# tyiannak/pyAudioAnalysis

Hardware: AMD Instinct MI355X
Metric: short-term frames/sec (34-feat, 16 kHz, 50 ms/25 ms) + HBM GB/s vs peak (higher is better)
Workload: dtype f64

## Files before the change

### pyaudioanalysis_amd/csrc/lib_host_api.hpp

```cpp
#pragma once
constexpr long long kRangedMinFrames = 65536;

static int run_host_st(const void *packed, const int64_t *offsets, int64_t n_clips, int sample_kind, double fs,
                       int window, int step, int deltas, double *out, const int64_t *out_offsets,
                       int64_t mid_ratio, int64_t mid_step, double *mid_out, const int64_t *mid_out_offsets) {
    if (!packed || !offsets) return fail(PAA_ERR_ARG, "null signal");
    { const int rc0 = ensure_init(); if (rc0) return rc0; }
    LaneGuard lane;
    const bool want_mid = mid_out != nullptr;
    if (want_mid && !deltas) return fail(PAA_ERR_ARG, "mid-term features are defined over the 68 delta rows");
    if (want_mid && mid_step < 1)
        return fail(PAA_ERR_ARG, "mid_step / short_step rounds to %lld: the reference loops forever "
                    "(MidTermFeatures.py:102,124)", (long long)mid_step);
    paa_plan *plan = nullptr;
    int rc;
    const long long frames_1 = (n_clips == 1) ? paa_num_frames(offsets[1] - offsets[0], window, step) : 0;
    const bool ranged = n_clips == 1 && out && !out_offsets && !want_mid && frames_1 >= kRangedMinFrames;
    {
        std::lock_guard<std::mutex> lk(g_mu);
        rc = plan_build(offsets, n_clips, sample_kind, fs, window, step, deltas, 0, &plan, ranged ? kCopyRanges : 1);
    }
    if (rc) return rc;
    std::unique_ptr<paa_plan, void (*)(paa_plan *)> guard(plan, plan_free_synced);
    const size_t esz = sample_kind == 0 ? 2 : (sample_kind == 2 ? 4 : 8);
    const long long base = offsets[0], n_total = offsets[n_clips] - base;
    if (base != 0) {
        for (auto &cd : plan->clips) cd.sample_off -= base;
        HIP_TRY(hipMemcpy(plan->d_clips, plan->clips.data(), plan->clips.size() * sizeof(ClipDev), hipMemcpyHostToDevice));
        std::vector<StatChunk> chunks;
        for (int64_t c = 0; c < n_clips; ++c)
            for (int i = 0; i < plan->clips[c].stat_count; ++i) {
                StatChunk ch; ch.start = plan->clips[c].sample_off + (long long)i * plan->stat_chunk;
                ch.len = (int)std::min<long long>(plan->stat_chunk, plan->clips[c].n - (long long)i * plan->stat_chunk);
                ch.clip = (int)c;
                chunks.push_back(ch);
            }
        if (!chunks.empty())
            HIP_TRY(hipMemcpy(plan->d_chunks, chunks.data(), chunks.size() * sizeof(StatChunk), hipMemcpyHostToDevice));
    }
    {
        std::lock_guard<std::mutex> lk(g_mu);
        if ((rc = scratch_reserve(lane.l->in, (size_t)n_total * esz + 64))) return rc;
        if ((rc = scratch_reserve(lane.l->out, (size_t)plan->out_doubles * 8))) return rc;
    }
    HIP_TRY(hipMemcpyAsync(lane.l->in.p, (const char *)packed + (size_t)base * esz, (size_t)n_total * esz,
                           hipMemcpyHostToDevice, cs()));
    const void *d_samples = lane.l->in.p;
    if (ranged && !plan->tiles_host.empty()) {
        double *d_out = (double *)lane.l->out.p;
        const long long T = plan->clips[0].T;
        const int F = plan->P.F;
        struct CopyStreamGuard { hipStream_t s; ~CopyStreamGuard() { if (s) (void)hipStreamSynchronize(s); } } copy_guard{lane.l->copy_stream};
        {
            std::lock_guard<std::mutex> lk(g_mu);
            if ((rc = launch_stats(plan, d_samples))) return rc;
        }
        long long first = 0;
        long long t_begin[kCopyRanges + 1];
        int used = 0;
        for (int r = 0; r < kCopyRanges && first < plan->n_tiles; ++r) {
            const long long t_target = (r == kCopyRanges - 1) ? T : T * (r + 1) / kCopyRanges;
            long long last = first;
            while (last < plan->n_tiles && (long long)plan->tiles_host[(size_t)last].t0 < t_target) ++last;
            if (last == first) continue;
            t_begin[used] = plan->tiles_host[(size_t)first].t0;
            {
                std::lock_guard<std::mutex> lk(g_mu);
                rc = kFamilies[plan->fam.family].execute(plan, d_samples, d_out, plan->d_tiles + first, last - first);
            }
            if (rc) return rc;
            HIP_TRY(hipEventRecord(lane.l->range_done[used], cs()));
            first = last;
            ++used;
        }
        t_begin[used] = T;
        for (int r = 0; r < used; ++r) {
            const long long a = t_begin[r], b = t_begin[r + 1];
            HIP_TRY(hipStreamWaitEvent(lane.l->copy_stream, lane.l->range_done[r], 0));
            HIP_TRY(hipMemcpy2DAsync(out + a, (size_t)T * 8, d_out + a, (size_t)T * 8, (size_t)(b - a) * 8, (size_t)F,
                                     hipMemcpyDeviceToHost, lane.l->copy_stream));
        }
        HIP_TRY(hipStreamSynchronize(lane.l->copy_stream));
        HIP_TRY(hipStreamSynchronize(cs()));
        return PAA_OK;
    }
    if ((rc = paa_plan_execute(plan, d_samples, (double *)lane.l->out.p))) return rc;
    if (want_mid) {
        const long long md = paa_plan_mid_doubles(plan, mid_step);
        {
            std::lock_guard<std::mutex> lk(g_mu);
            if ((rc = scratch_reserve(lane.l->mid, (size_t)md * 8))) return rc;
        }
        if ((rc = paa_plan_mid_execute(plan, (const double *)lane.l->out.p, mid_ratio, mid_step, (double *)lane.l->mid.p))) return rc;
        long long o = 0;
        for (int64_t c = 0; c < n_clips; ++c) {
            const long long cnt = 2LL * plan->P.F * paa_num_mid_windows(plan->clips[c].T, mid_step);
            double *dst = mid_out + (mid_out_offsets ? mid_out_offsets[c] : o);
            HIP_TRY(hipMemcpyAsync(dst, (double *)lane.l->mid.p + o, (size_t)cnt * 8, hipMemcpyDeviceToHost, cs()));
            o += cnt;
        }
    }
    if (out) {
        if (!out_offsets) {
            HIP_TRY(hipMemcpyAsync(out, lane.l->out.p, (size_t)plan->out_doubles * 8, hipMemcpyDeviceToHost, cs()));
        } else {
            int64_t c = 0;
            while (c < n_clips) {
                int64_t e = c;
                long long cnt = 0;
                while (e < n_clips && out_offsets[e] - out_offsets[c] == plan->clips[e].out_off - plan->clips[c].out_off) {
                    cnt = plan->clips[e].out_off - plan->clips[c].out_off + (long long)plan->P.F * plan->clips[e].T;
                    ++e;
                }
                HIP_TRY(hipMemcpyAsync(out + out_offsets[c], (double *)lane.l->out.p + plan->clips[c].out_off,
                                       (size_t)cnt * 8, hipMemcpyDeviceToHost, cs()));
                c = e;
            }
        }
    }
    HIP_TRY(hipStreamSynchronize(cs()));
    return PAA_OK;
}

extern "C" int paa_st_features_i16(const int16_t *signal, int64_t n, double fs, int window, int step, int deltas,
                                   double *out) {
    if (!out) return fail(PAA_ERR_ARG, "null out");
    const int64_t off[2] = {0, n};
    return run_host_st(signal, off, 1, 0, fs, window, step, deltas, out, nullptr, 0, 0, nullptr, nullptr);
}
extern "C" int paa_st_features_f64(const double *signal, int64_t n, double fs, int window, int step, int deltas,
                                   double *out) {
    if (!out) return fail(PAA_ERR_ARG, "null out");
    const int64_t off[2] = {0, n};
    return run_host_st(signal, off, 1, 1, fs, window, step, deltas, out, nullptr, 0, 0, nullptr, nullptr);
}
extern "C" int paa_st_features_stereo_i16(const int16_t *interleaved, int64_t n, double fs, int window, int step,
                                          int deltas, double *out) {
    if (!out) return fail(PAA_ERR_ARG, "null out");
// ... 190 lines not shown
```

### pyaudioanalysis_amd/csrc/lib_plan.hpp

```cpp
#pragma once
#ifndef PAA_STAT_CHUNK
#define PAA_STAT_CHUNK 131072
#endif
constexpr int kStatChunk = PAA_STAT_CHUNK;
static int stat_chunk_for(long long total_samples, int num_cu) {
    const long long blocks = (total_samples + kStatChunk - 1) / kStatChunk;
    if (blocks < num_cu) {
        const long long len = ((total_samples + 4LL * num_cu - 1) / (4LL * num_cu) + 63) / 64 * 64;
        return (int)std::min<long long>(kStatChunk, std::max<long long>(len, 4096));
    }
    const long long want = (blocks + num_cu - 1) / num_cu * num_cu;
    const long long len = ((total_samples + want - 1) / want + 63) / 64 * 64;
    return (int)std::min<long long>(kStatChunk, std::max<long long>(len, 4096));
}

static int choose_run_cap(const std::vector<ClipDev> &clips, int quantum, int min_run, int max_run, int halo, int wg_runs,
                          int num_cu, int shrink = 0) {
    std::map<long long, long long> hist;
    for (const ClipDev &c : clips)
        if (c.T > 0) ++hist[c.T];
    if (hist.empty()) return max_run;
    long long best_cost = -1;
    int best = max_run;
    for (int cap = max_run / quantum * quantum; cap >= min_run; cap -= quantum) {
// ... 19 lines not shown

static bool balanced_runs(const std::vector<ClipDev> &clips, int run, int quantum, int shrink, int wg_runs, int num_cu, int min_run,
                          std::vector<std::vector<int>> &lens) {
    if (wg_runs < 2 || quantum < 1 || shrink < 0 || (shrink > 0 && shrink >= quantum)) return false;
    long long total = 0, runs = 0;
    std::vector<long long> need(clips.size(), 0);
    for (size_t c = 0; c < clips.size(); ++c) {
        const long long T = clips[c].T;
        if (T <= 0) continue;
        total += T;
        const long long len = clip_run_length(T, run, quantum), later = std::max<long long>(len - shrink, 1);
        need[c] = (T <= len) ? 1 : 1 + (T - len + later - 1) / later;
        runs += need[c];
    }
    const long long slots = (long long)num_cu * wg_runs;
    if (runs >= slots || (runs + wg_runs - 1) / wg_runs > num_cu || total < slots * min_run) return false;
    std::vector<long long> k(clips.size(), 0);
    long long given = 0;
    for (size_t c = 0; c < clips.size(); ++c) {
        const long long T = clips[c].T;
        if (T <= 0) continue;
        k[c] = std::max<long long>(need[c], std::min<long long>(slots * T / total, std::max<long long>(T / min_run, 1)));
        given += k[c];
    }
    if (given > slots) return false;
    std::vector<std::vector<int>> out(clips.size());
    const int per = (wg_runs % 4 == 0) ? wg_runs / 4 : 0;
    long long first_tile = 0;
    for (size_t c = 0; c < clips.size(); ++c) {
        const long long T = clips[c].T, kc = k[c];
        if (T <= 0) continue;
        const long long iters = (T + (kc - 1) * shrink + quantum - 1) / quantum, base = iters / kc, longs = iters % kc;
        if (base < 1 || (base + (longs ? 1 : 0)) * quantum > run) return false;
        std::vector<int> &l = out[c];
        l.assign((size_t)kc, (int)(base * quantum));
        std::vector<std::pair<long long, long long>> order;
        order.reserve((size_t)kc);
        for (long long i = 0; i < kc; ++i) {
            const long long tile = first_tile + i, w = tile % wg_runs, j = tile / wg_runs;
            order.emplace_back(per ? (j * 4 + w % 4) * per + w / 4 : tile, i);
        }
        std::sort(order.begin(), order.end());
        for (long long u = 0; u < kc; ++u)
            if ((u + 1) * longs / kc > u * longs / kc) l[(size_t)order[(size_t)u].second] += quantum;
        long long sum = 0;
        for (size_t i = 0; i < l.size(); ++i) { if (i > 0) l[i] -= shrink; sum += l[i]; }
        l.back() -= (int)(sum - T);
        if (l.back() <= 0) return false;
        first_tile += kc;
    }
    lens.swap(out);
    return true;
}

struct FamilyChoice {
    int family = -1;
    FastLaunch fl;
    ct::CtLaunch cl;
    tri::TriLaunch trl;
    mix::MixLayout ml;
    blu::BluLayout bl;
    GenLayout gl;
    wg::WgLayout wl;
    size_t lds = 0;
    std::string kernel_name;
    unsigned char *d_blob = nullptr;
};

struct paa_plan {
    long long n_clips = 0;
    int sample_kind = 0;
    int mode = 0;
    int row_width = 0;
    std::vector<ClipDev> clips;
    std::vector<long long> alloc_rows;
    long long total_frames = 0, out_doubles = 0;
    TableSet *tab = nullptr;
    int stat_chunk = kStatChunk;
    PlanDev P;
    ClipDev *d_clips = nullptr;
    ClipNorm *d_norms = nullptr;
    Tile *d_tiles = nullptr;
    StatChunk *d_chunks = nullptr;
    void *d_psum = nullptr, *d_pmin = nullptr, *d_pmax = nullptr;
    long long *d_mid_off = nullptr;
    FamilyChoice fam;
    bool blob_cached = false;
    void *d_block = nullptr;
    void *d_big = nullptr;
    size_t big_bytes = 0;
    std::vector<wg::FrameRef> wg_frames;
    std::vector<std::pair<long long, long long>> wg_chunks;
    wg::FrameRef *d_wg_frames = nullptr;
    std::vector<wg::FrameRef> wg_tasks;
    std::vector<std::pair<long long, long long>> wg_task_chunks;
    wg::FrameRef *d_wg_tasks = nullptr;
    long long wg_rows = 0;
    long long mid_off_step = -1;
    long long n_tiles = 0, n_chunks = 0;
    std::vector<Tile> tiles_host;
};

static std::atomic<int> g_live_plans{0};
static void plan_free(paa_plan *p) {
    if (!p) return;
    --g_live_plans;
    pool_free(p->d_block);
    pool_free(p->d_mid_off);
    pool_free(p->d_wg_frames);
    pool_free(p->d_wg_tasks);
    if (!p->blob_cached) pool_free(p->fam.d_blob);
    if (p->d_big) (void)hipFree(p->d_big);
    delete p;
}

static void plan_free_synced(paa_plan *p) {
    if (!p) return;
    if (cs()) (void)hipStreamSynchronize(cs());
    plan_free(p);
}

static int launch_stats(paa_plan *p, const void *d_packed) {
    if (p->n_chunks > 0) {
        if (p->sample_kind == 0)
            hipLaunchKernelGGL(clip_stats_i16_kernel, dim3((unsigned)p->n_chunks), dim3(256), 0, cs(),
                               (const int16_t *)d_packed, p->d_chunks, (long long *)p->d_psum, (int *)p->d_pmin,
                               (int *)p->d_pmax);
        else if (p->sample_kind == 2)
            hipLaunchKernelGGL(clip_stats_stereo_kernel, dim3((unsigned)p->n_chunks), dim3(256), 0, cs(),
                               (const stereo16 *)d_packed, p->d_chunks, (long long *)p->d_psum, (int *)p->d_pmin,
                               (int *)p->d_pmax);
        else
            hipLaunchKernelGGL(clip_stats_f64_kernel, dim3((unsigned)p->n_chunks), dim3(256), 0, cs(),
                               (const double *)d_packed, p->d_chunks, (double *)p->d_psum, (double *)p->d_pmin,
                               (double *)p->d_pmax);
    }
    const unsigned gb = (unsigned)p->n_clips;
    if (p->P.norms_inline) {
        HIP_TRY(hipGetLastError());
        return PAA_OK;
    }
    if (p->sample_kind == 1)
        hipLaunchKernelGGL((clip_params_kernel<double, double>), dim3(gb), dim3(64), 0, cs(), p->d_clips,
                           p->n_clips, (const double *)p->d_psum, (const double *)p->d_pmin,
                           (const double *)p->d_pmax, sample_scale<double>(), p->P.W, p->d_norms);
    else
        hipLaunchKernelGGL((clip_params_kernel<long long, int>), dim3(gb), dim3(64), 0, cs(), p->d_clips,
                           p->n_clips, (const long long *)p->d_psum, (const int *)p->d_pmin, (const int *)p->d_pmax,
                           p->sample_kind == 2 ? sample_scale<stereo16>() : sample_scale<int16_t>(), p->P.W, p->d_norms);
    HIP_TRY(hipGetLastError());
    return PAA_OK;
}

template <typename T>
static int run_big(paa_plan *p, const void *d_packed, double *d_out) {
    const PlanDev &P = p->P;
    const long long Nc = P.Nc, Nf = P.Nf;
    const size_t per_frame = (size_t)Nc * 32 + (size_t)Nf * 8 + 24;
    long long maxT = 0;
    for (auto &cd : p->clips) maxT = std::max<long long>(maxT, cd.T);
    long long C = (long long)std::max<size_t>(1, ((size_t)1 << 30) / per_frame);
    C = std::min<long long>(std::min<long long>(C, 65535), std::max<long long>(maxT, 1));
    const size_t need = (size_t)C * Nc * 32 + (size_t)(C + 1) * Nf * 8 + (size_t)C * 24 + 256;
    if (need > p->big_bytes) {
        if (p->d_big) { HIP_TRY(hipStreamSynchronize(cs())); (void)hipFree(p->d_big); p->d_big = nullptr; }
        HIP_TRY(hipMalloc(&p->d_big, need));
        p->big_bytes = need;
    }
    double2 *bufA = reinterpret_cast<double2 *>(p->d_big);
    double2 *bufB = bufA + C * Nc;
    double *spec = reinterpret_cast<double *>(bufB + C * Nc);
    double *tfeat = spec + (C + 1) * Nf;
    const unsigned gx = (unsigned)std::min<long long>(64, (std::max<long long>(Nc, P.W) + 255) / 256);
    for (long long c = 0; c < p->n_clips; ++c) {
        const ClipDev &cd = p->clips[c];
        const T *x0 = (const T *)d_packed + cd.sample_off + P.frame_origin;
        double *oc = d_out + cd.out_off;
        long long prev_n = 0;
        for (long long t0 = 0; t0 < cd.T; t0 += C) {
            const long long n = std::min<long long>(C, cd.T - t0);
            if (t0 > 0 && P.mode != 1)
                HIP_TRY(hipMemcpyAsync(spec, spec + prev_n * Nf, (size_t)Nf * 8, hipMemcpyDeviceToDevice, cs()));
            hipLaunchKernelGGL(big_load_kernel<T>, dim3(gx, (unsigned)n), dim3(256), 0, cs(), P, x0, t0, ClipNorm(),
                               p->d_norms, (int)c, bufA);
            if (P.mode == 0)
                hipLaunchKernelGGL(big_time_kernel, dim3((unsigned)n), dim3(64), 0, cs(), P, bufA, tfeat);
            double2 *src = bufA, *dst = bufB;
            int Ns = 1;
            for (int q = 0; q < P.n_pass; ++q) {
                hipLaunchKernelGGL(big_pass_kernel, dim3(gx, (unsigned)n), dim3(256), 0, cs(), (int)Nc, P.radix[q], Ns,
                                   P.tw, src, dst);
                Ns *= P.radix[q];
                std::swap(src, dst);
            }
            if (P.mode == 1) {
                hipLaunchKernelGGL(big_post_kernel, dim3(gx, (unsigned)n), dim3(256), 0, cs(), P, src, oc, t0);
            } else {
                hipLaunchKernelGGL(big_post_kernel, dim3(gx, (unsigned)n), dim3(256), 0, cs(), P, src, spec, 1LL);
                hipLaunchKernelGGL(big_feat_kernel, dim3((unsigned)n), dim3(64), 0, cs(), P, spec, tfeat, t0,
                                   (long long)cd.T, oc);
            }
            HIP_TRY(hipGetLastError());
            prev_n = n;
        }
        if (P.mode == 0 && P.deltas) {
            const long long items = (long long)kBase * cd.T;
            hipLaunchKernelGGL(big_delta_kernel, dim3((unsigned)((items + 255) / 256)), dim3(256), 0, cs(),
                               (long long)cd.T, oc);
            HIP_TRY(hipGetLastError());
        }
    }
    return PAA_OK;
}

struct ProfScope {
    hipEvent_t stop = nullptr;
    int begin() {
        if (!(g_prof && (g_prof_seen++ % g_prof) == 0)) return PAA_OK;
        if (g_prof_used == g_prof_ev.size()) {
            hipEvent_t a, b;
            HIP_TRY(hipEventCreate(&a));
            HIP_TRY(hipEventCreate(&b));
            g_prof_ev.emplace_back(a, b);
        }
        const hipEvent_t start = g_prof_ev[g_prof_used].first;
        stop = g_prof_ev[g_prof_used].second;
        ++g_prof_used;
        HIP_TRY(hipEventRecord(start, cs()));
        return PAA_OK;
    }
    ~ProfScope() { if (stop) (void)hipEventRecord(stop, cs()); }
// ... 143 lines not shown
    long long out_off = 0, total_frames = 0, n_chunks = 0;
    p->stat_chunk = stat_chunk_for(offsets[n_clips] - offsets[0], g_num_cu);
    const int kChunk = p->stat_chunk;
    for (int64_t c = 0; c < n_clips; ++c) {
        const long long n = offsets[c + 1] - offsets[c];
        if (n < 0) return fail(PAA_ERR_ARG, "offsets must be non-decreasing (clip %lld)", (long long)c);
        ClipDev &cd = p->clips[c];
        cd.sample_off = offsets[c];
        cd.n = n;
        cd.out_off = out_off;
        long long T = 0, rows = 0;
        if (mode == 0) {
            T = paa_num_frames(n, window, step);
            if (T < 1)
                return fail(PAA_ERR_TOO_SHORT, "need at least one array to concatenate (clip %lld has %lld samples, "
                            "window %d)", (long long)c, n, window);
            rows = T;
            out_off += (long long)F * T;
        } else {
            int64_t filled = 0;
            rows = (mode == 1) ? paa_spectrogram_rows(n, window, step, &filled)
                               : paa_chromagram_rows(n, window, step, &filled);
            if (rows < 1)
                return fail(PAA_ERR_TOO_SHORT, "signal too short for window %d / step %d (clip %lld, %lld samples)",
                            window, step, (long long)c, n);
            long long full = 0;
            for (long long pos = window; pos + window <= n && full < filled; pos += step) ++full;
            T = full;
            out_off += rows * p->row_width;
        }
        if (T > 0x7fffffffLL) return fail(PAA_ERR_ARG, "clip %lld has too many frames", (long long)c);
        p->alloc_rows[c] = rows;
        cd.T = (int)T;
        cd.stat_first = (int)n_chunks;
        cd.stat_count = (int)((n + kChunk - 1) / kChunk);
        cd.pad = 0;
        n_chunks += cd.stat_count;
        total_frames += T;
    }
    p->total_frames = total_frames;
    p->out_doubles = out_off;
    p->n_chunks = n_chunks;

    PlanDev &P = p->P;
    memset(&P, 0, sizeof(P));
    P.W = window; P.S = step; P.Nf = Nf; P.Nc = tab->fft.len; P.even = tab->fft.even;
    P.n_pass = (int)tab->fft.radix.size();
    if (P.n_pass > 24) return fail(PAA_ERR_UNSUPPORTED, "window %d needs more than 24 FFT passes", window);
    for (int i = 0; i < P.n_pass; ++i) P.radix[i] = tab->fft.radix[i];
    P.tw = tab->d_tw; P.post = tab->d_post;
    P.mel_lo = tab->d_mel_lo; P.mel_cnt = tab->d_mel_cnt; P.mel_off = tab->d_mel_off; P.mel_w = tab->d_mel_w;
    P.dct = tab->d_dct; P.ch_start = tab->d_ch_start; P.ch_src = tab->d_ch_src; P.ch_w = tab->d_ch_w;
    P.fs = fs; P.deltas = deltas ? 1 : 0; P.F = F;
    P.blk_t = window / 10; P.blk_f = Nf / 10;
    P.mode = mode;
    P.frame_origin = (mode == 0) ? 0 : window;
    { const char *dbg = experiment_env("PAA_KERNEL_DEBUG"); P.debug = dbg ? atoi(dbg) : 0; }

    FamilyCtx fc{p.get(), tab, fs, window, step, deltas, mode, sample_kind, F, total_frames, ranges};
    if ((rc = choose_family(fc))) return rc;
    const Family &fam = kFamilies[p->fam.family];
    std::vector<Tile> tiles;
    if ((rc = fam.work(fc, tiles))) return rc;
    p->n_tiles = (long long)tiles.size();
    if (ranges > 1 && fam.ranged) p->tiles_host = tiles;
    if (p->n_tiles > 0x7fffffffLL || n_chunks > 0x7fffffffLL || n_clips > 0x7fffffffLL)
        return fail(PAA_ERR_UNSUPPORTED, "batch too large for one launch (%lld runs, %lld statistics chunks, %lld clips)",
                    p->n_tiles, n_chunks, (long long)n_clips);
    std::vector<StatChunk> chunks;
    chunks.reserve((size_t)n_chunks);
    for (int64_t c = 0; c < n_clips; ++c)
        for (int i = 0; i < p->clips[c].stat_count; ++i) {
            StatChunk ch; ch.start = p->clips[c].sample_off + (long long)i * kChunk;
            ch.len = (int)std::min<long long>(kChunk, p->clips[c].n - (long long)i * kChunk);
            ch.clip = (int)c;
            chunks.push_back(ch);
        }
    {
        const size_t nch = (size_t)std::max<long long>(n_chunks, 1);
        const size_t o_clips = 0, o_tiles = o_clips + up256(p->clips.size() * sizeof(ClipDev));
        const size_t o_chunks = o_tiles + up256(std::max<size_t>(tiles.size(), 1) * sizeof(Tile));
        const size_t o_norms = o_chunks + up256(std::max<size_t>(chunks.size(), 1) * sizeof(StatChunk));
        const size_t o_sum = o_norms + up256((size_t)n_clips * sizeof(ClipNorm));
        const size_t o_min = o_sum + up256(nch * 8), o_max = o_min + up256(nch * 8), total = o_max + up256(nch * 8);
        if ((rc = pool_alloc(&p->d_block, total))) return rc;
        std::vector<unsigned char> stage(o_norms, 0);
        memcpy(stage.data() + o_clips, p->clips.data(), p->clips.size() * sizeof(ClipDev));
        if (!tiles.empty()) memcpy(stage.data() + o_tiles, tiles.data(), tiles.size() * sizeof(Tile));
        if (!chunks.empty()) memcpy(stage.data() + o_chunks, chunks.data(), chunks.size() * sizeof(StatChunk));
        HIP_TRY(hipMemcpy(p->d_block, stage.data(), o_norms, hipMemcpyHostToDevice));
        unsigned char *b = reinterpret_cast<unsigned char *>(p->d_block);
        p->d_clips = reinterpret_cast<ClipDev *>(b + o_clips);
        p->d_tiles = reinterpret_cast<Tile *>(b + o_tiles);
        p->d_chunks = reinterpret_cast<StatChunk *>(b + o_chunks);
        p->d_norms = reinterpret_cast<ClipNorm *>(b + o_norms);
        p->d_psum = b + o_sum; p->d_pmin = b + o_min; p->d_pmax = b + o_max;
    }
    P.st_sum = p->d_psum; P.st_min = p->d_pmin; P.st_max = p->d_pmax;
    P.st_scale = sample_kind == 1 ? sample_scale<double>() : (sample_kind == 2 ? sample_scale<stereo16>() : sample_scale<int16_t>());
    P.norms_inline = (fam.norms_inline && mode != 2) ? 1 : 0;
    *out = p.release();
    return PAA_OK;
}

extern "C" int paa_plan_execute(paa_plan_t *plan, const void *d_packed, double *d_out) {
    if (!plan || !d_packed || !d_out) return fail(PAA_ERR_ARG, "null plan / buffer");
    { const int rc_init = ensure_init(); if (rc_init) return rc_init; }
    std::lock_guard<std::mutex> lk(g_mu);
    int rc = comm_wait_buffer_free(d_out);
    if (rc) return rc;
    rc = launch_stats(plan, d_packed);
    if (rc) return rc;
    return kFamilies[plan->fam.family].execute(plan, d_packed, d_out, plan->d_tiles, plan->n_tiles);
}

extern "C" int paa_plan_create(const int64_t *offsets, int64_t n_clips, int sample_kind, double fs, int window,
                               int step, int deltas, paa_plan_t **out_plan) {
    std::lock_guard<std::mutex> lk(g_mu);
    return plan_build(offsets, n_clips, sample_kind, fs, window, step, deltas, 0, out_plan);
}

extern "C" int paa_plan_create_mode(const int64_t *offsets, int64_t n_clips, int sample_kind, double fs, int window,
                                    int step, int mode, paa_plan_t **out_plan) {
    if (mode < 0 || mode > 2) return fail(PAA_ERR_ARG, "mode must be 0 (features), 1 (spectrogram) or 2 (chromagram)");
    std::lock_guard<std::mutex> lk(g_mu);
    return plan_build(offsets, n_clips, sample_kind, fs, window, step, 0, mode, out_plan);
}

extern "C" int paa_plan_destroy(paa_plan_t *plan) {
    if (g_device.load() >= 0) (void)ensure_init();
    std::lock_guard<std::mutex> lk(g_mu);
    if (cs()) (void)hipStreamSynchronize(cs());
    plan_free(plan);
    return PAA_OK;
}

extern "C" int64_t paa_plan_total_frames(const paa_plan_t *plan) { return plan ? plan->total_frames : 0; }
extern "C" int64_t paa_plan_out_doubles(const paa_plan_t *plan) { return plan ? plan->out_doubles : 0; }
extern "C" const char *paa_plan_kernel_name(const paa_plan_t *plan) { return plan ? plan->fam.kernel_name.c_str() : ""; }

extern "C" int paa_plan_out_offsets(const paa_plan_t *plan, int64_t *out_offsets) {
    if (!plan || !out_offsets) return fail(PAA_ERR_ARG, "null plan / buffer");
    for (long long c = 0; c < plan->n_clips; ++c) out_offsets[c] = plan->clips[c].out_off;
    return PAA_OK;
}

extern "C" int64_t paa_plan_mid_doubles(const paa_plan_t *plan, int64_t mid_step_ratio) {
    if (!plan || mid_step_ratio < 1) return 0;
    long long tot = 0;
    for (long long c = 0; c < plan->n_clips; ++c)
        tot += 2LL * plan->P.F * paa_num_mid_windows(plan->clips[c].T, mid_step_ratio);
    return tot;
}

extern "C" int paa_plan_mid_execute(paa_plan_t *plan, const double *d_st, int64_t mid_ratio, int64_t mid_step_ratio,
                                    double *d_mid) {
    if (!plan || !d_st || !d_mid) return fail(PAA_ERR_ARG, "null plan / buffer");
    { const int rc_init = ensure_init(); if (rc_init) return rc_init; }
    if (plan->mode != 0) return fail(PAA_ERR_ARG, "mid-term statistics need a feature plan");
    if (mid_step_ratio < 1)
        return fail(PAA_ERR_ARG, "mid_step / short_step rounds to %lld: the reference loops forever "
                    "(MidTermFeatures.py:102,124)", (long long)mid_step_ratio);
    std::lock_guard<std::mutex> lk(g_mu);
    { const int rc_w = comm_wait_buffer_free(d_mid); if (rc_w) return rc_w; }
    long long maxM = 0;
    if (plan->mid_off_step != mid_step_ratio) {
        std::vector<long long> off(plan->n_clips);
        long long o = 0;
        for (long long c = 0; c < plan->n_clips; ++c) {
            off[c] = o;
            o += 2LL * plan->P.F * paa_num_mid_windows(plan->clips[c].T, mid_step_ratio);
        }
        if (cs()) HIP_TRY(hipStreamSynchronize(cs()));
        int rc = upload_pooled(&plan->d_mid_off, off.data(), off.size());
        if (rc) return rc;
        plan->mid_off_step = mid_step_ratio;
    }
    for (long long c = 0; c < plan->n_clips; ++c)
        maxM = std::max<long long>(maxM, paa_num_mid_windows(plan->clips[c].T, mid_step_ratio));
    const long long items = (long long)plan->P.F * maxM;
    const int bpc = (int)((items + 15) / 16);
    const long long grid = plan->n_clips * bpc;
    if (grid > 0x7fffffffLL) return fail(PAA_ERR_UNSUPPORTED, "mid-term grid too large");
    hipLaunchKernelGGL(mid_stats_kernel, dim3((unsigned)grid), dim3(256), 0, cs(), plan->d_clips, plan->d_mid_off,
                       d_st, plan->P.F, (long long)mid_ratio, (long long)mid_step_ratio, bpc, d_mid);
    HIP_TRY(hipGetLastError());
    return PAA_OK;
}

extern "C" int paa_plan_beat_execute(paa_plan_t *plan, const double *d_st, double window_size, double *d_beat) {
    if (!plan || !d_st || !d_beat) return fail(PAA_ERR_ARG, "null plan / buffer");
    if (plan->mode != 0) return fail(PAA_ERR_ARG, "beat extraction needs a feature plan");
    if (!(window_size > 0)) return fail(PAA_ERR_ARG, "window_size must be positive");
    { const int rc_init = ensure_init(); if (rc_init) return rc_init; }
    const int max_beat = (int)nearbyint(2.0 / window_size);
    if (max_beat < 1) return fail(PAA_ERR_ARG, "attempt to get argmax of an empty sequence (beat histogram of %d bins)", max_beat);
    if (max_beat > 4096) return fail(PAA_ERR_UNSUPPORTED, "beat histogram of %d bins", max_beat);
    std::lock_guard<std::mutex> lk(g_mu);
    { const int rc_w = comm_wait_buffer_free(d_beat); if (rc_w) return rc_w; }
    const size_t lds = (size_t)kBeatRows * (kBeatTile + 1) * 8 + (size_t)kBeatRows * max_beat * 4;
    if (lds > 160 * 1024)
        return fail(PAA_ERR_UNSUPPORTED, "beat histogram of %d bins needs %zu bytes of LDS (160 KB per workgroup)", max_beat, lds);
    if (lds > 64 * 1024)
        HIP_TRY(hipFuncSetAttribute(reinterpret_cast<const void *>(&beat_kernel), hipFuncAttributeMaxDynamicSharedMemorySize, (int)lds));
    hipLaunchKernelGGL(beat_kernel, dim3((unsigned)plan->n_clips), dim3(64), lds, cs(), plan->d_clips, d_st,
                       window_size, max_beat, d_beat);
    HIP_TRY(hipGetLastError());
    return PAA_OK;
}

struct DeltaPlanCache {
    std::vector<int64_t> frames;
    DeltaTile *d_tiles = nullptr;
    long long n_tiles = 0;
};
// ... 40 lines not shown
```

### pyaudioanalysis_amd/csrc/paa_lib.hip

```cpp
#include <dlfcn.h>
#include <hip/hip_runtime.h>

#include <algorithm>
#include <atomic>
#include <cstdarg>
#include <cstdio>
#include <cmath>
#include <cstring>
#include <limits>
#include <map>
#include <memory>
#include <condition_variable>
#include <mutex>
#include <string>
#include <tuple>
#include <utility>
#include <vector>

#include "../../include/paa_hip.h"
#define PAA_NO_HOST_LAUNCHERS
#include "family_launch.hpp"
#include "kernels_aux.hpp"
#include "kernels_big.hpp"
#include "kernels_wg.hpp"
#include "kernels_wgr.hpp"
#include "kernels_wgs.hpp"
#include "kernels_sim.hpp"
#include "kernels_svm.hpp"
#include "tables.hpp"

using namespace paa;

static thread_local char g_err[512] = "";

static int fail(int code, const char *fmt, ...) {
    va_list ap;
    va_start(ap, fmt);
    vsnprintf(g_err, sizeof(g_err), fmt, ap);
    va_end(ap);
    return code;
}

#define HIP_TRY(expr)                                                                         \
    do {                                                                                      \
        hipError_t e_ = (expr);                                                               \
        if (e_ != hipSuccess)                                                                 \
            return fail(e_ == hipErrorOutOfMemory ? PAA_ERR_OOM : PAA_ERR_HIP, "%s: %s (%s:%d)", \
                        #expr, hipGetErrorString(e_), __FILE__, __LINE__);                    \
    } while (0)

struct TableSet {
    double fs;
    int window;
    FftPlan fft;
    MelTable mel;
    ChromaTable chroma;
    double2 *d_tw = nullptr, *d_post = nullptr;
    int *d_mel_lo = nullptr, *d_mel_cnt = nullptr, *d_mel_off = nullptr;
    double *d_mel_w = nullptr, *d_dct = nullptr;
    int *d_ch_start = nullptr, *d_ch_src = nullptr;
    double *d_ch_w = nullptr;
    FastTables fast;
    std::map<std::tuple<int, int, int>, std::shared_ptr<struct FamilyChoice>> choices;
};

struct Scratch {
    void *p = nullptr;
    size_t cap = 0;
};
struct GlobalScratch : Scratch {
    GlobalScratch *next;
    GlobalScratch();
};
static GlobalScratch *g_global_scratch = nullptr;
inline GlobalScratch::GlobalScratch() : next(g_global_scratch) { g_global_scratch = this; }

static std::mutex g_mu;
static std::mutex g_api_mu;
static std::atomic<int> g_device{-1};
static std::recursive_mutex g_init_mu;
static hipStream_t g_main_stream = nullptr;
static hipEvent_t g_ev0 = nullptr, g_ev1 = nullptr;
static std::map<std::pair<double, int>, std::unique_ptr<TableSet>> g_tables;
constexpr int kCopyRanges = 4;
struct Lane {
    hipStream_t stream = nullptr;
    hipStream_t copy_stream = nullptr;
    hipEvent_t range_done[kCopyRanges] = {nullptr, nullptr, nullptr, nullptr};
    Scratch in, out, mid;
    bool busy = false;
};
constexpr int kLanes = 4;
static Lane g_lanes[kLanes];
static std::mutex g_lane_mu;
static std::condition_variable g_lane_cv;
static int g_lanes_active = 0, g_lanes_peak = 0;
static thread_local Lane *tl_lane = nullptr;
static inline hipStream_t cs() { return tl_lane ? tl_lane->stream : g_main_stream; }
struct LaneGuard {
    Lane *l = nullptr;
    bool nested = false;
    LaneGuard() {
        if (tl_lane) { l = tl_lane; nested = true; return; }
        std::unique_lock<std::mutex> lk(g_lane_mu);
        for (;;) {
            for (int i = 0; i < kLanes; ++i)
                if (!g_lanes[i].busy && g_lanes[i].stream) { l = &g_lanes[i]; break; }
            if (l) break;
            g_lane_cv.wait(lk);
        }
        l->busy = true;
        g_lanes_peak = std::max(g_lanes_peak, ++g_lanes_active);
        tl_lane = l;
    }
    ~LaneGuard() {
        if (nested || !l) return;
        tl_lane = nullptr;
        {
            std::lock_guard<std::mutex> lk(g_lane_mu);
            l->busy = false;
            --g_lanes_active;
        }
        g_lane_cv.notify_one();
    }
};
static GlobalScratch g_sim_z, g_sim_small, g_sim_cand, g_sim_in, g_sim_out, g_sim_filt;
static GlobalScratch g_svc_sums;
static GlobalScratch g_forest_scratch;
static int g_force_generic = 0;
static int g_f800_waves = 8;
static int g_num_cu = 256;
static int g_prof = 0;
static long long g_prof_seen = 0;
static std::vector<std::pair<hipEvent_t, hipEvent_t>> g_prof_ev;
static size_t g_prof_used = 0;
static double g_prof_ms = 0.0;
static long long g_prof_n = 0;

static int comm_wait_buffer_free(const void *d_out);
static void comm_forget_buffer(const void *ptr);
static int comm_sync();

static thread_local int tl_device = -1;
static int ensure_init() {
    if (g_device.load(std::memory_order_acquire) < 0) {
        std::lock_guard<std::recursive_mutex> lk(g_init_mu);
        if (g_device.load(std::memory_order_acquire) < 0) {
            const int rc = paa_init(0);
            if (rc) return rc;
        }
    }
    const int dev = g_device.load(std::memory_order_acquire);
    if (tl_device != dev) {
        HIP_TRY(hipSetDevice(dev));
        tl_device = dev;
    }
    return PAA_OK;
}

template <typename T>
static int upload(T **dst, const void *src, size_t count) {
    if (*dst) (void)hipFree(*dst);
    *dst = nullptr;
    if (count == 0) count = 1;
    HIP_TRY(hipMalloc((void **)dst, count * sizeof(T)));
    if (src) HIP_TRY(hipMemcpy(*dst, src, count * sizeof(T), hipMemcpyHostToDevice));
    return PAA_OK;
}

static void scratch_release(Scratch &s) {
    if (s.p) (void)hipFree(s.p);
    s.p = nullptr;
    s.cap = 0;
}
static int scratch_reserve(Scratch &s, size_t bytes) {
    if (bytes <= s.cap) return PAA_OK;
    scratch_release(s);
    size_t want = bytes + bytes / 8 + 4096;
    HIP_TRY(hipMalloc(&s.p, want));
    s.cap = want;
    return PAA_OK;
}

struct DevPool {
    std::mutex mu;
    std::multimap<size_t, void *> idle;
    std::map<void *, size_t> size_of;
    size_t idle_bytes = 0;
};
static DevPool g_pool;
static int pool_alloc(void **out, size_t bytes) {
    size_t cls = 4096;
    while (cls < bytes) cls <<= 1;
    {
        std::lock_guard<std::mutex> lk(g_pool.mu);
        auto it = g_pool.idle.find(cls);
        if (it != g_pool.idle.end()) {
            *out = it->second;
            g_pool.idle.erase(it);
            g_pool.idle_bytes -= cls;
            return PAA_OK;
        }
    }
    HIP_TRY(hipMalloc(out, cls));
    std::lock_guard<std::mutex> lk(g_pool.mu);
    g_pool.size_of[*out] = cls;
    return PAA_OK;
}
static void pool_free(void *p) {
    if (!p) return;
    std::unique_lock<std::mutex> lk(g_pool.mu);
    auto it = g_pool.size_of.find(p);
    if (it == g_pool.size_of.end()) { lk.unlock(); (void)hipFree(p); return; }
    if (g_pool.idle_bytes + it->second <= ((size_t)256 << 20)) {
        g_pool.idle.emplace(it->second, p);
        g_pool.idle_bytes += it->second;
        return;
    }
    g_pool.size_of.erase(it);
    lk.unlock();
    (void)hipFree(p);
// ... 33 lines not shown
        t->window = window;
        build_fft_plan(window, t->fft);
        int rc;
        double dct[kNumMfcc * kNumMel];
        build_dct(dct);
        if ((rc = upload(&t->d_tw, t->fft.tw.data(), t->fft.tw.size() / 2)) ||
            (rc = upload(&t->d_post, t->fft.post.data(), t->fft.post.size() / 2)) ||
            (rc = upload(&t->d_dct, dct, (size_t)kNumMfcc * kNumMel))) {
            free_tables(*t);
            return rc;
        }
        it = g_tables.emplace(key, std::move(t)).first;
    }
    TableSet *t = it->second.get();
    const int nfft = window / 2;
    if (need_mel && !t->d_mel_w) {
        int rc = build_mel(fs, nfft, t->mel);
        if (rc == PAA_ERR_MEL_INDEX)
            return fail(rc, "mel filter bank indexes bin >= num_fft=%d at fs=%g (IndexError in the reference, "
                            "ShortTermFeatures.py:230-231)", nfft, fs);
        if ((rc = upload(&t->d_mel_lo, t->mel.lo.data(), t->mel.lo.size()))) return rc;
        if ((rc = upload(&t->d_mel_cnt, t->mel.cnt.data(), t->mel.cnt.size()))) return rc;
        if ((rc = upload(&t->d_mel_off, t->mel.off.data(), t->mel.off.size()))) return rc;
        if ((rc = upload(&t->d_mel_w, t->mel.w.data(), t->mel.w.size()))) return rc;
    }
    if (need_chroma && !t->d_ch_w) {
        int rc = build_chroma(fs, nfft, t->chroma);
        if (rc == PAA_ERR_CHROMA_VALUE)
            return fail(rc, "shape mismatch: chroma slot exceeds num_fft=%d (ValueError in the reference, "
                            "ShortTermFeatures.py:293)", nfft);
        if (rc == PAA_ERR_CHROMA_INDEX)
            return fail(rc, "chroma slot out of bounds for num_fft=%d (IndexError in the reference, "
                            "ShortTermFeatures.py:291)", nfft);
        if ((rc = upload(&t->d_ch_start, t->chroma.class_start, 13))) return rc;
        if ((rc = upload(&t->d_ch_src, t->chroma.src.data(), t->chroma.src.size()))) return rc;
        if ((rc = upload(&t->d_ch_w, t->chroma.w.data(), t->chroma.w.size()))) return rc;
    }
    *out = t;
    return PAA_OK;
}

#include "lib_model.hpp"
#include "lib_plan.hpp"
#include "lib_similarity.hpp"

extern "C" const char *paa_version(void) { return "paa_hip 0.1 (gfx950)"; }
extern "C" const char *paa_last_error(void) { return g_err; }

extern "C" int paa_device_count(void) {
    int n = 0;
    hipError_t e = hipGetDeviceCount(&n);
    if (e != hipSuccess) return fail(PAA_ERR_HIP, "hipGetDeviceCount: %s", hipGetErrorString(e));
    return n;
}

extern "C" int paa_device_bus_id(char *out, int capacity) {
    if (!out || capacity < 16) return fail(PAA_ERR_ARG, "bus id buffer too small");
    int rc = ensure_init();
    if (rc) return rc;
    HIP_TRY(hipDeviceGetPCIBusId(out, capacity, g_device.load()));
    return PAA_OK;
}

extern "C" int paa_init(int device_id) {
    std::lock_guard<std::recursive_mutex> init_lock(g_init_mu);
    if (g_device == device_id && g_main_stream) {
        if (tl_device != device_id) { HIP_TRY(hipSetDevice(device_id)); tl_device = device_id; }
        return PAA_OK;
    }
    int n = 0;
    hipError_t e = hipGetDeviceCount(&n);
    if (e != hipSuccess || n < 1)
        return fail(PAA_ERR_HIP, "no HIP device (%s); this library has no CPU path", hipGetErrorString(e));
    if (device_id < 0 || device_id >= n) return fail(PAA_ERR_ARG, "device %d out of range (%d devices)", device_id, n);
    if (g_device >= 0 && g_device != device_id) {
        if (g_live_plans.load() > 0)
            return fail(PAA_ERR_ARG, "paa_init(%d): %d plan(s) of device %d are still alive; destroy them first",
                        device_id, g_live_plans.load(), g_device.load());
        paa_shutdown();
    }
    HIP_TRY(hipSetDevice(device_id));
    tl_device = device_id;
    if (!g_main_stream) HIP_TRY(hipStreamCreateWithFlags(&g_main_stream, hipStreamNonBlocking));
    for (int i = 0; i < kLanes; ++i) {
        if (!g_lanes[i].stream) HIP_TRY(hipStreamCreateWithFlags(&g_lanes[i].stream, hipStreamNonBlocking));
        if (!g_lanes[i].copy_stream) HIP_TRY(hipStreamCreateWithFlags(&g_lanes[i].copy_stream, hipStreamNonBlocking));
        for (int k = 0; k < kCopyRanges; ++k)
            if (!g_lanes[i].range_done[k]) HIP_TRY(hipEventCreateWithFlags(&g_lanes[i].range_done[k], hipEventDisableTiming));
    }
    if (!g_ev0) HIP_TRY(hipEventCreate(&g_ev0));
    if (!g_ev1) HIP_TRY(hipEventCreate(&g_ev1));
    {
        int ncu = 0;
        if (hipDeviceGetAttribute(&ncu, hipDeviceAttributeMultiprocessorCount, device_id) == hipSuccess && ncu > 0) g_num_cu = ncu;
    }
    const char *fg = experiment_env("PAA_HIP_FORCE_GENERIC");
    g_force_generic = (fg && fg[0] == '1') ? 1 : 0;
    const char *fw = experiment_env("PAA_F800_WAVES");
    g_f800_waves = (fw && fw[0] == '4') ? 4 : 8;
    g_device.store(device_id, std::memory_order_release);
    return PAA_OK;
}

extern "C" void paa_shutdown(void) {
    std::lock_guard<std::recursive_mutex> init_lock(g_init_mu);
    if (g_device < 0) return;
    (void)paa_comm_destroy();
    if (g_main_stream) (void)hipStreamSynchronize(g_main_stream);
    for (auto &kv : g_tables) free_tables(*kv.second);
    g_tables.clear();
    pool_release_all();
    for (GlobalScratch *s = g_global_scratch; s; s = s->next) scratch_release(*s);
    for (Lane &ln : g_lanes) {
        if (ln.stream) { (void)hipStreamSynchronize(ln.stream); (void)hipStreamDestroy(ln.stream); ln.stream = nullptr; }
        if (ln.copy_stream) { (void)hipStreamSynchronize(ln.copy_stream); (void)hipStreamDestroy(ln.copy_stream); ln.copy_stream = nullptr; }
        for (hipEvent_t &ev : ln.range_done) { if (ev) (void)hipEventDestroy(ev); ev = nullptr; }
        for (Scratch *s : {&ln.in, &ln.out, &ln.mid}) scratch_release(*s);
    }
    if (g_ev0) (void)hipEventDestroy(g_ev0);
    if (g_ev1) (void)hipEventDestroy(g_ev1);
    if (g_main_stream) (void)hipStreamDestroy(g_main_stream);
    g_ev0 = g_ev1 = nullptr;
    g_main_stream = nullptr;
    ++lds_attr_generation();
    g_device.store(-1, std::memory_order_release);
}

extern "C" int paa_dev_alloc(size_t bytes, void **out_ptr) {
    int rc = ensure_init();
    if (rc) return rc;
    if (!out_ptr) return fail(PAA_ERR_ARG, "null out_ptr");
    HIP_TRY(hipMalloc(out_ptr, bytes ? bytes : 1));
    return PAA_OK;
}
extern "C" int paa_dev_free(void *ptr) {
    if (ptr) {
        comm_forget_buffer(ptr);
        HIP_TRY(hipFree(ptr));
    }
    return PAA_OK;
}
extern "C" int paa_memcpy_d2d(void *dst, const void *src, size_t bytes) {
    int rc = ensure_init();
    if (rc) return rc;
    HIP_TRY(hipMemcpyAsync(dst, src, bytes, hipMemcpyDeviceToDevice, cs()));
    return PAA_OK;
}
extern "C" int paa_memcpy_h2d(void *dst, const void *src, size_t bytes) {
    int rc = ensure_init();
    if (rc) return rc;
    HIP_TRY(hipMemcpyAsync(dst, src, bytes, hipMemcpyHostToDevice, cs()));
    HIP_TRY(hipStreamSynchronize(cs()));
    return PAA_OK;
}
extern "C" int paa_memcpy_d2h(void *dst, const void *src, size_t bytes) {
    int rc = ensure_init();
    if (rc) return rc;
    if ((rc = comm_sync())) return rc;
    HIP_TRY(hipMemcpyAsync(dst, src, bytes, hipMemcpyDeviceToHost, cs()));
    HIP_TRY(hipStreamSynchronize(cs()));
    return PAA_OK;
}
extern "C" int paa_memcpy_d2h_compute(void *dst, const void *src, size_t bytes) {
    int rc = ensure_init();
    if (rc) return rc;
    HIP_TRY(hipMemcpyAsync(dst, src, bytes, hipMemcpyDeviceToHost, cs()));
    HIP_TRY(hipStreamSynchronize(cs()));
    return PAA_OK;
}
extern "C" int paa_dev_sync(void) {
    int rc = ensure_init();
    if (rc) return rc;
    HIP_TRY(hipStreamSynchronize(cs()));
    return comm_sync();
}
extern "C" int paa_timer_start(void) {
    int rc = ensure_init();
    if (rc) return rc;
    HIP_TRY(hipEventRecord(g_ev0, cs()));
    return PAA_OK;
}
extern "C" int paa_timer_stop(float *ms) {
    int rc = ensure_init();
    if (rc) return rc;
    HIP_TRY(hipEventRecord(g_ev1, cs()));
    HIP_TRY(hipEventSynchronize(g_ev1));
    HIP_TRY(hipEventElapsedTime(ms, g_ev0, g_ev1));
    return PAA_OK;
}

extern "C" int paa_prof_enable(int on) {
    std::lock_guard<std::mutex> lk(g_mu);
    g_prof = on > 0 ? on : 0;
    g_prof_seen = 0;
    return PAA_OK;
}
extern "C" int paa_prof_read(double *total_ms, int64_t *launches) {
    int rc = ensure_init();
    if (rc) return rc;
    std::lock_guard<std::mutex> lk(g_mu);
    HIP_TRY(hipStreamSynchronize(cs()));
    for (size_t i = 0; i < g_prof_used; ++i) {
        float ms = 0.f;
        HIP_TRY(hipEventElapsedTime(&ms, g_prof_ev[i].first, g_prof_ev[i].second));
        g_prof_ms += ms;
        ++g_prof_n;
    }
    g_prof_used = 0;
    if (total_ms) *total_ms = g_prof_ms;
    if (launches) *launches = g_prof_n;
    g_prof_ms = 0.0;
    g_prof_n = 0;
    return PAA_OK;
}

extern "C" int64_t paa_num_frames(int64_t n, int window, int step) {
    if (window < 1 || step < 1 || n < window) return 0;
    return (n - window) / step + 1;
}
extern "C" int64_t paa_num_mid_windows(int64_t T, int64_t mid_step_ratio) {
    if (T < 1 || mid_step_ratio < 1) return 0;
    return (T + mid_step_ratio - 1) / mid_step_ratio;
}
extern "C" int64_t paa_spectrogram_rows(int64_t n, int window, int step, int64_t *filled) {
    if (filled) *filled = 0;
    if (window < 1 || step < 1) return 0;
    const int64_t num = n - window;
    const int64_t rows = (num >= 0 ? num / step : -((-num) / step)) + 1;
    int64_t f = 0;
    for (int64_t p = window; p < n - window + 1; p += step) ++f;
    if (filled) *filled = f;
    return rows;
}
extern "C" int64_t paa_chromagram_rows(int64_t n, int window, int step, int64_t *filled) {
    if (filled) *filled = 0;
    if (window < 1 || step < 1) return 0;
    const int64_t num = n - step - window;
    const int64_t rows = (num >= 0 ? num / step : -((-num) / step)) + 1;
    int64_t f = 0;
    for (int64_t p = window; p < n - step; p += step) ++f;
    if (filled) *filled = f;
    return rows;
}

#include "lib_host_api.hpp"
#include "lib_svc.hpp"
#include "lib_knn.hpp"
#include "lib_forest.hpp"
#include "lib_hmm.hpp"
#include "lib_diar.hpp"

#include "comm_rccl.hpp"

#include "lib_debug.hpp"
```

Before: 557.9 million.

## Overlap clip-stats kernels on a side stream with double-buffered stat sets

Adds a dedicated stats stream and two ping-ponged stat buffers per plan so the clip-statistics reduction of the next call can run concurrently with the feature kernels of the previous call on the main stream. Events chain the dependencies, and the chain is broken whenever the main stream is touched through cs() or when the input overlaps the previous output. The intent is to hide the stats pass latency in repeated device-resident calls, at the cost of extra event bookkeeping and subtle ordering rules.

Result: slower. 533.6 million (-4.4%).

```diff
diff --git a/pyaudioanalysis_amd/csrc/lib_host_api.hpp b/pyaudioanalysis_amd/csrc/lib_host_api.hpp
--- a/pyaudioanalysis_amd/csrc/lib_host_api.hpp
+++ b/pyaudioanalysis_amd/csrc/lib_host_api.hpp
@@ -53,7 +53,7 @@
         struct CopyStreamGuard { hipStream_t s; ~CopyStreamGuard() { if (s) (void)hipStreamSynchronize(s); } } copy_guard{lane.l->copy_stream};
         {
             std::lock_guard<std::mutex> lk(g_mu);
-            if ((rc = launch_stats(plan, d_samples))) return rc;
+            if ((rc = launch_stats(plan, d_samples, plan->sets[0], cs()))) return rc;
         }
         long long first = 0;
         long long t_begin[kCopyRanges + 1];
diff --git a/pyaudioanalysis_amd/csrc/lib_plan.hpp b/pyaudioanalysis_amd/csrc/lib_plan.hpp
--- a/pyaudioanalysis_amd/csrc/lib_plan.hpp
+++ b/pyaudioanalysis_amd/csrc/lib_plan.hpp
@@ -125,7 +125,13 @@
     ClipNorm *d_norms = nullptr;
     Tile *d_tiles = nullptr;
     StatChunk *d_chunks = nullptr;
-    void *d_psum = nullptr, *d_pmin = nullptr, *d_pmax = nullptr;
+    struct StatSet {
+        void *d_psum = nullptr, *d_pmin = nullptr, *d_pmax = nullptr;
+        hipEvent_t written = nullptr;
+        hipEvent_t read_done = nullptr;
+        bool in_use = false;
+    } sets[2];
+    unsigned long long n_overlapped = 0;
     long long *d_mid_off = nullptr;
     FamilyChoice fam;
     bool blob_cached = false;
@@ -144,10 +150,25 @@
     std::vector<Tile> tiles_host;
 };
 
+struct ChainLink {
+    const paa_plan *plan = nullptr;
+    hipEvent_t done = nullptr;
+    const char *out_lo = nullptr, *out_hi = nullptr;
+};
+static ChainLink g_chain[2];
+static void chain_forget() {
+    g_chain[0] = g_chain[1] = ChainLink();
+    g_chain_open.store(false, std::memory_order_relaxed);
+}
+
 static std::atomic<int> g_live_plans{0};
 static void plan_free(paa_plan *p) {
     if (!p) return;
     --g_live_plans;
+    for (paa_plan::StatSet &st : p->sets) {
+        if (st.written) (void)hipEventDestroy(st.written);
+        if (st.read_done) (void)hipEventDestroy(st.read_done);
+    }
     pool_free(p->d_block);
     pool_free(p->d_mid_off);
     pool_free(p->d_wg_frames);
@@ -160,23 +181,24 @@
 static void plan_free_synced(paa_plan *p) {
     if (!p) return;
     if (cs()) (void)hipStreamSynchronize(cs());
+    if (p->n_overlapped && g_stats_stream) (void)hipStreamSynchronize(g_stats_stream);
     plan_free(p);
 }
 
-static int launch_stats(paa_plan *p, const void *d_packed) {
+static int launch_stats(paa_plan *p, const void *d_packed, const paa_plan::StatSet &st, hipStream_t s) {
     if (p->n_chunks > 0) {
         if (p->sample_kind == 0)
-            hipLaunchKernelGGL(clip_stats_i16_kernel, dim3((unsigned)p->n_chunks), dim3(256), 0, cs(),
-                               (const int16_t *)d_packed, p->d_chunks, (long long *)p->d_psum, (int *)p->d_pmin,
-                               (int *)p->d_pmax);
+            hipLaunchKernelGGL(clip_stats_i16_kernel, dim3((unsigned)p->n_chunks), dim3(256), 0, s,
+                               (const int16_t *)d_packed, p->d_chunks, (long long *)st.d_psum, (int *)st.d_pmin,
+                               (int *)st.d_pmax);
         else if (p->sample_kind == 2)
-            hipLaunchKernelGGL(clip_stats_stereo_kernel, dim3((unsigned)p->n_chunks), dim3(256), 0, cs(),
-                               (const stereo16 *)d_packed, p->d_chunks, (long long *)p->d_psum, (int *)p->d_pmin,
-                               (int *)p->d_pmax);
+            hipLaunchKernelGGL(clip_stats_stereo_kernel, dim3((unsigned)p->n_chunks), dim3(256), 0, s,
+                               (const stereo16 *)d_packed, p->d_chunks, (long long *)st.d_psum, (int *)st.d_pmin,
+                               (int *)st.d_pmax);
         else
-            hipLaunchKernelGGL(clip_stats_f64_kernel, dim3((unsigned)p->n_chunks), dim3(256), 0, cs(),
-                               (const double *)d_packed, p->d_chunks, (double *)p->d_psum, (double *)p->d_pmin,
-                               (double *)p->d_pmax);
+            hipLaunchKernelGGL(clip_stats_f64_kernel, dim3((unsigned)p->n_chunks), dim3(256), 0, s,
+                               (const double *)d_packed, p->d_chunks, (double *)st.d_psum, (double *)st.d_pmin,
+                               (double *)st.d_pmax);
     }
     const unsigned gb = (unsigned)p->n_clips;
     if (p->P.norms_inline) {
@@ -184,12 +206,12 @@
         return PAA_OK;
     }
     if (p->sample_kind == 1)
-        hipLaunchKernelGGL((clip_params_kernel<double, double>), dim3(gb), dim3(64), 0, cs(), p->d_clips,
-                           p->n_clips, (const double *)p->d_psum, (const double *)p->d_pmin,
-                           (const double *)p->d_pmax, sample_scale<double>(), p->P.W, p->d_norms);
+        hipLaunchKernelGGL((clip_params_kernel<double, double>), dim3(gb), dim3(64), 0, s, p->d_clips,
+                           p->n_clips, (const double *)st.d_psum, (const double *)st.d_pmin,
+                           (const double *)st.d_pmax, sample_scale<double>(), p->P.W, p->d_norms);
     else
-        hipLaunchKernelGGL((clip_params_kernel<long long, int>), dim3(gb), dim3(64), 0, cs(), p->d_clips,
-                           p->n_clips, (const long long *)p->d_psum, (const int *)p->d_pmin, (const int *)p->d_pmax,
+        hipLaunchKernelGGL((clip_params_kernel<long long, int>), dim3(gb), dim3(64), 0, s, p->d_clips,
+                           p->n_clips, (const long long *)st.d_psum, (const int *)st.d_pmin, (const int *)st.d_pmax,
                            p->sample_kind == 2 ? sample_scale<stereo16>() : sample_scale<int16_t>(), p->P.W, p->d_norms);
     HIP_TRY(hipGetLastError());
     return PAA_OK;
@@ -499,7 +521,8 @@
         const size_t o_chunks = o_tiles + up256(std::max<size_t>(tiles.size(), 1) * sizeof(Tile));
         const size_t o_norms = o_chunks + up256(std::max<size_t>(chunks.size(), 1) * sizeof(StatChunk));
         const size_t o_sum = o_norms + up256((size_t)n_clips * sizeof(ClipNorm));
-        const size_t o_min = o_sum + up256(nch * 8), o_max = o_min + up256(nch * 8), total = o_max + up256(nch * 8);
+        const size_t o_min = o_sum + up256(nch * 8), o_max = o_min + up256(nch * 8), set_bytes = o_max + up256(nch * 8) - o_sum;
+        const size_t total = o_sum + 2 * set_bytes;
         if ((rc = pool_alloc(&p->d_block, total))) return rc;
         std::vector<unsigned char> stage(o_norms, 0);
         memcpy(stage.data() + o_clips, p->clips.data(), p->clips.size() * sizeof(ClipDev));
@@ -511,12 +534,48 @@
         p->d_tiles = reinterpret_cast<Tile *>(b + o_tiles);
         p->d_chunks = reinterpret_cast<StatChunk *>(b + o_chunks);
         p->d_norms = reinterpret_cast<ClipNorm *>(b + o_norms);
-        p->d_psum = b + o_sum; p->d_pmin = b + o_min; p->d_pmax = b + o_max;
-    }
-    P.st_sum = p->d_psum; P.st_min = p->d_pmin; P.st_max = p->d_pmax;
+        for (int k = 0; k < 2; ++k) {
+            paa_plan::StatSet &st = p->sets[k];
+            st.d_psum = b + o_sum + k * set_bytes; st.d_pmin = b + o_min + k * set_bytes; st.d_pmax = b + o_max + k * set_bytes;
+        }
+    }
+    P.st_sum = p->sets[0].d_psum; P.st_min = p->sets[0].d_pmin; P.st_max = p->sets[0].d_pmax;
     P.st_scale = sample_kind == 1 ? sample_scale<double>() : (sample_kind == 2 ? sample_scale<stereo16>() : sample_scale<int16_t>());
     P.norms_inline = (fam.norms_inline && mode != 2) ? 1 : 0;
     *out = p.release();
+    return PAA_OK;
+}
+
+static int run_overlapped(paa_plan *p, const void *d_packed, double *d_out) {
+    paa_plan::StatSet &st = p->sets[p->n_overlapped & 1];
+    if (!st.written) HIP_TRY(hipEventCreateWithFlags(&st.written, hipEventDisableTiming));
+    if (!st.read_done) HIP_TRY(hipEventCreateWithFlags(&st.read_done, hipEventDisableTiming));
+    ++p->n_overlapped;
+    const size_t esz = p->sample_kind == 0 ? 2 : (p->sample_kind == 2 ? 4 : 8);
+    const char *in_lo = (const char *)d_packed + (size_t)p->clips.front().sample_off * esz;
+    const char *in_hi = (const char *)d_packed + (size_t)(p->clips.back().sample_off + p->clips.back().n) * esz;
+    const bool open = g_chain_open.load(std::memory_order_relaxed) && (in_hi <= g_chain[0].out_lo || in_lo >= g_chain[0].out_hi);
+    if (open) {
+        if (g_chain[1].done) HIP_TRY(hipStreamWaitEvent(g_stats_stream, g_chain[1].done, 0));
+        if (st.in_use && st.read_done != g_chain[1].done) HIP_TRY(hipStreamWaitEvent(g_stats_stream, st.read_done, 0));
+    } else {
+        HIP_TRY(hipEventRecord(g_stats_fence, g_main_stream));
+        HIP_TRY(hipStreamWaitEvent(g_stats_stream, g_stats_fence, 0));
+        g_chain[0] = g_chain[1] = ChainLink();
+    }
+    int rc = launch_stats(p, d_packed, st, g_stats_stream);
+    if (rc) return rc;
+    HIP_TRY(hipEventRecord(st.written, g_stats_stream));
+    HIP_TRY(hipStreamWaitEvent(g_main_stream, st.written, 0));
+    p->P.st_sum = st.d_psum; p->P.st_min = st.d_pmin; p->P.st_max = st.d_pmax;
+    rc = kFamilies[p->fam.family].execute(p, d_packed, d_out, p->d_tiles, p->n_tiles);
+    if (rc) return rc;
+    HIP_TRY(hipEventRecord(st.read_done, g_main_stream));
+    st.in_use = true;
+    g_chain[1] = g_chain[0];
+    g_chain[0].plan = p; g_chain[0].done = st.read_done;
+    g_chain[0].out_lo = (const char *)d_out; g_chain[0].out_hi = (const char *)d_out + (size_t)p->out_doubles * 8;
+    g_chain_open.store(true, std::memory_order_relaxed);
     return PAA_OK;
 }
 
@@ -526,7 +585,10 @@
     std::lock_guard<std::mutex> lk(g_mu);
     int rc = comm_wait_buffer_free(d_out);
     if (rc) return rc;
-    rc = launch_stats(plan, d_packed);
+    if (!tl_lane && plan->P.norms_inline && plan->n_chunks > 0 && plan->n_tiles > 0) return run_overlapped(plan, d_packed, d_out);
+    const hipStream_t s = cs();
+    plan->P.st_sum = plan->sets[0].d_psum; plan->P.st_min = plan->sets[0].d_pmin; plan->P.st_max = plan->sets[0].d_pmax;
+    rc = launch_stats(plan, d_packed, plan->sets[0], s);
     if (rc) return rc;
     return kFamilies[plan->fam.family].execute(plan, d_packed, d_out, plan->d_tiles, plan->n_tiles);
 }
@@ -548,6 +610,10 @@
     if (g_device.load() >= 0) (void)ensure_init();
     std::lock_guard<std::mutex> lk(g_mu);
     if (cs()) (void)hipStreamSynchronize(cs());
+    if (plan && plan->n_overlapped) {
+        if (g_stats_stream) (void)hipStreamSynchronize(g_stats_stream);
+        chain_forget();
+    }
     plan_free(plan);
     return PAA_OK;
 }
diff --git a/pyaudioanalysis_amd/csrc/paa_lib.hip b/pyaudioanalysis_amd/csrc/paa_lib.hip
--- a/pyaudioanalysis_amd/csrc/paa_lib.hip
+++ b/pyaudioanalysis_amd/csrc/paa_lib.hip
@@ -80,6 +80,9 @@
 static std::atomic<int> g_device{-1};
 static std::recursive_mutex g_init_mu;
 static hipStream_t g_main_stream = nullptr;
+static hipStream_t g_stats_stream = nullptr;
+static hipEvent_t g_stats_fence = nullptr;
+static std::atomic<bool> g_chain_open{false};
 static hipEvent_t g_ev0 = nullptr, g_ev1 = nullptr;
 static std::map<std::pair<double, int>, std::unique_ptr<TableSet>> g_tables;
 constexpr int kCopyRanges = 4;
@@ -96,7 +99,11 @@
 static std::condition_variable g_lane_cv;
 static int g_lanes_active = 0, g_lanes_peak = 0;
 static thread_local Lane *tl_lane = nullptr;
-static inline hipStream_t cs() { return tl_lane ? tl_lane->stream : g_main_stream; }
+static inline hipStream_t cs() {
+    if (tl_lane) return tl_lane->stream;
+    g_chain_open.store(false, std::memory_order_relaxed);
+    return g_main_stream;
+}
 struct LaneGuard {
     Lane *l = nullptr;
     bool nested = false;
@@ -137,6 +144,7 @@
 static double g_prof_ms = 0.0;
 static long long g_prof_n = 0;
 
+static void chain_forget();
 static int comm_wait_buffer_free(const void *d_out);
 static void comm_forget_buffer(const void *ptr);
 static int comm_sync();
@@ -336,6 +344,8 @@
     HIP_TRY(hipSetDevice(device_id));
     tl_device = device_id;
     if (!g_main_stream) HIP_TRY(hipStreamCreateWithFlags(&g_main_stream, hipStreamNonBlocking));
+    if (!g_stats_stream) HIP_TRY(hipStreamCreateWithFlags(&g_stats_stream, hipStreamNonBlocking));
+    if (!g_stats_fence) HIP_TRY(hipEventCreateWithFlags(&g_stats_fence, hipEventDisableTiming));
     for (int i = 0; i < kLanes; ++i) {
         if (!g_lanes[i].stream) HIP_TRY(hipStreamCreateWithFlags(&g_lanes[i].stream, hipStreamNonBlocking));
         if (!g_lanes[i].copy_stream) HIP_TRY(hipStreamCreateWithFlags(&g_lanes[i].copy_stream, hipStreamNonBlocking));
@@ -361,6 +371,7 @@
     if (g_device < 0) return;
     (void)paa_comm_destroy();
     if (g_main_stream) (void)hipStreamSynchronize(g_main_stream);
+    if (g_stats_stream) (void)hipStreamSynchronize(g_stats_stream);
     for (auto &kv : g_tables) free_tables(*kv.second);
     g_tables.clear();
     pool_release_all();
@@ -373,9 +384,12 @@
     }
     if (g_ev0) (void)hipEventDestroy(g_ev0);
     if (g_ev1) (void)hipEventDestroy(g_ev1);
+    if (g_stats_fence) (void)hipEventDestroy(g_stats_fence);
+    if (g_stats_stream) (void)hipStreamDestroy(g_stats_stream);
     if (g_main_stream) (void)hipStreamDestroy(g_main_stream);
-    g_ev0 = g_ev1 = nullptr;
-    g_main_stream = nullptr;
+    g_ev0 = g_ev1 = g_stats_fence = nullptr;
+    g_main_stream = g_stats_stream = nullptr;
+    chain_forget();
     ++lds_attr_generation();
     g_device.store(-1, std::memory_order_release);
 }
@@ -425,7 +439,9 @@
 extern "C" int paa_dev_sync(void) {
     int rc = ensure_init();
     if (rc) return rc;
-    HIP_TRY(hipStreamSynchronize(cs()));
+    const hipStream_t s = cs();
+    HIP_TRY(hipStreamSynchronize(s));
+    if (s == g_main_stream && g_stats_stream) HIP_TRY(hipStreamSynchronize(g_stats_stream));
     return comm_sync();
 }
 extern "C" int paa_timer_start(void) {
```
